# Keluaa/Armon.jl

Hardware: AMD Instinct MI355X
Metric: Mcells/sec per sweep (fp64) (higher is better)
Workload: dtype f64; 1 GPU; Sod 16384x16384 fp64, GAD+minmod+euler_2nd, Sequential X,Y splitting, nghost 4, 1x1 tiles of 16384x16384 cells (strong scaling); arithmetic=tuned (shared 1-ulp reciprocals + FMA; within the reference's golden tolerance), cells_per_gpu=268435456, transport=single block, device=AMD GPU gfx950 (gfx950:sramecc+:xnack-, 256 CUs), halo_exchange_downgraded=False, full=False

## Files before the change

### armon.jl_amd/csrc/common.hpp

```cpp
#pragma once

#include <hip/hip_runtime.h>

#include <cstdarg>
#include <cstdint>
#include <cstdio>
#include <cstring>

#include "../../include/armon_hip.h"

struct armon_graph;
struct armon_ctx {
    int device = 0;
    hipStream_t stream = nullptr;
    bool owns_stream = false;
    double* partials = nullptr;
    size_t partials_cap = 0;
    double* scalars = nullptr;
    double* host_scalars = nullptr;
    hipEvent_t ev_start = nullptr, ev_stop = nullptr;
    hipEvent_t* ev_pool = nullptr;
    int n_cu = 256;
    int tune_xs_niter = 0;
    int tune_y_seg = 0;
    int tune_align = 1;
    int tune_y_cols1 = 0;
    int tune_x_xcd = -1;
    int tune_x_rows = 0;
    int tune_copy_nt = 0;
    int tune_y_sx = 0;
    int64_t seg_nx = -1, seg_ny = -1;
    int seg_lag = -1, seg_cols = -1, seg_value = 0;
    int live_graphs = 0;
    armon_graph* graphs = nullptr;
    bool capturing = false;
};

namespace armon {

void set_error(const char* fmt, ...);

inline int fail_hip(hipError_t e, const char* what)
{
    set_error("%s: %s", what, hipGetErrorString(e));
    return ARMON_ERR_HIP;
}

#define ARMON_HIP_TRY(expr)                                             \
    do {                                                                \
        hipError_t e_ = (expr);                                         \
        if (e_ != hipSuccess) return ::armon::fail_hip(e_, #expr);      \
    } while (0)

#define ARMON_REQUIRE(cond, ...)                                        \
    do {                                                                \
        if (!(cond)) {                                                  \
            ::armon::set_error(__VA_ARGS__);                            \
            return ARMON_ERR_INVALID_ARG;                               \
        }                                                               \
    } while (0)

inline int check_launch(const char* name)
{
    hipError_t e = hipGetLastError();
    if (e != hipSuccess) {
// ... 30 lines not shown
```

### armon.jl_amd/csrc/context.hip

```cpp
#include "common.hpp"

#include <cstdlib>

namespace armon {

static thread_local char g_error[512] = "";

void set_error(const char* fmt, ...)
{
    va_list ap;
    va_start(ap, fmt);
    vsnprintf(g_error, sizeof(g_error), fmt, ap);
    va_end(ap);
}

int ensure_partials(armon_ctx* ctx, size_t n)
{
    if (n <= ctx->partials_cap) return ARMON_OK;
    ARMON_REQUIRE(!ctx->capturing, "the reduction scratch would have to grow (%zu -> %zu doubles) inside a stream capture: "
                  "run this launch once before armon_hip_graph_begin", ctx->partials_cap, n);
    ARMON_REQUIRE(ctx->live_graphs == 0, "the reduction scratch would have to grow (%zu -> %zu doubles) while %d captured graph(s) of "
                  "this context point into it: destroy them first, or run the larger launch before capturing",
                  ctx->partials_cap, n, ctx->live_graphs);
    ARMON_HIP_TRY(hipStreamSynchronize(ctx->stream));
// ... 37 lines not shown
        set_error("no HIP device available (%s)", e != hipSuccess ? hipGetErrorString(e) : "count = 0");
        return ARMON_ERR_NO_DEVICE;
    }
    ARMON_REQUIRE(device_id >= 0 && device_id < n, "device_id %d out of range [0,%d)", device_id, n);
    ARMON_HIP_TRY(hipSetDevice(device_id));

    hipDeviceProp_t prop;
    ARMON_HIP_TRY(hipGetDeviceProperties(&prop, device_id));
    if (strncmp(prop.gcnArchName, "gfx950", 6) != 0) {
        set_error("device %d is %s; this library holds gfx950 code objects only", device_id, prop.gcnArchName);
        return ARMON_ERR_NO_DEVICE;
    }

    armon_ctx* ctx = new armon_ctx();
    ctx->device = device_id;
    ctx->n_cu = prop.multiProcessorCount;
    if (stream) {
        ctx->stream = (hipStream_t)stream;
        ctx->owns_stream = false;
    } else {
        e = hipStreamCreateWithFlags(&ctx->stream, hipStreamNonBlocking);
        if (e != hipSuccess) { delete ctx; return fail_hip(e, "hipStreamCreate"); }
        ctx->owns_stream = true;
    }
    if ((e = hipMalloc((void**)&ctx->scalars, 16 * sizeof(double))) != hipSuccess ||
        (e = hipHostMalloc((void**)&ctx->host_scalars, 16 * sizeof(double), hipHostMallocDefault)) != hipSuccess ||
        (e = hipEventCreate(&ctx->ev_start)) != hipSuccess ||
        (e = hipEventCreate(&ctx->ev_stop)) != hipSuccess) {
        armon_hip_destroy(ctx);
        return fail_hip(e, "context allocation");
    }
    int rc = ensure_partials(ctx, 8192);
    if (rc != ARMON_OK) { armon_hip_destroy(ctx); return rc; }
    for (const char* knob : {"ARMON_XS_NITER", "ARMON_Y_SEG", "ARMON_SWEEP_ALIGN", "ARMON_Y_COLS1", "ARMON_X_XCD", "ARMON_X_ROWS", "ARMON_Y_SX", "ARMON_COPY_NT"}) {
        const char* v = getenv(knob);
        if (v && *v) (void)armon_hip_set_tuning(ctx, knob, atoi(v));
    }
    *out = ctx;
    return ARMON_OK;
}

int armon_hip_set_tuning(armon_ctx* ctx, const char* knob, int value)
{
    ARMON_REQUIRE(ctx && knob, "NULL argument");
    if (!strcmp(knob, "ARMON_XS_NITER")) ctx->tune_xs_niter = value > 0 ? value : 0;
    else if (!strcmp(knob, "ARMON_Y_SEG")) ctx->tune_y_seg = value > 0 ? value : 0;
    else if (!strcmp(knob, "ARMON_SWEEP_ALIGN")) ctx->tune_align = value < 0 ? 1 : (value != 0);
    else if (!strcmp(knob, "ARMON_Y_COLS1")) ctx->tune_y_cols1 = value > 0;
    else if (!strcmp(knob, "ARMON_X_XCD")) ctx->tune_x_xcd = value < 0 ? -1 : (value > 0);
    else if (!strcmp(knob, "ARMON_X_ROWS")) ctx->tune_x_rows = (value == 1 || value == 2) ? value : 0;
    else if (!strcmp(knob, "ARMON_Y_SX")) ctx->tune_y_sx = (value == 1 || value == 2) ? value : 0;
    else if (!strcmp(knob, "ARMON_COPY_NT")) ctx->tune_copy_nt = value & 3;
    else ARMON_REQUIRE(false, "unknown tuning knob '%s'", knob);
    return ARMON_OK;
}

int armon_hip_get_tuning(armon_ctx* ctx, const char* knob, int* value)
{
    ARMON_REQUIRE(ctx && knob && value, "NULL argument");
    if (!strcmp(knob, "ARMON_XS_NITER")) *value = ctx->tune_xs_niter;
    else if (!strcmp(knob, "ARMON_Y_SEG")) *value = ctx->tune_y_seg;
    else if (!strcmp(knob, "ARMON_SWEEP_ALIGN")) *value = ctx->tune_align;
    else if (!strcmp(knob, "ARMON_Y_COLS1")) *value = ctx->tune_y_cols1;
    else if (!strcmp(knob, "ARMON_X_XCD")) *value = ctx->tune_x_xcd;
    else if (!strcmp(knob, "ARMON_X_ROWS")) *value = ctx->tune_x_rows;
    else if (!strcmp(knob, "ARMON_Y_SX")) *value = ctx->tune_y_sx;
    else if (!strcmp(knob, "ARMON_COPY_NT")) *value = ctx->tune_copy_nt;
    else if (!strcmp(knob, "Y_RUN_ROWS")) *value = ctx->tune_y_seg > 0 ? ctx->tune_y_seg : ctx->seg_value;
    else ARMON_REQUIRE(false, "unknown tuning knob '%s'", knob);
    return ARMON_OK;
}

int armon_hip_destroy(armon_ctx* ctx)
{
    if (!ctx) return ARMON_OK;
    (void)hipSetDevice(ctx->device);
    if (ctx->stream) (void)hipStreamSynchronize(ctx->stream);
    disown_graphs(ctx);
    if (ctx->partials) (void)hipFree(ctx->partials);
    if (ctx->scalars) (void)hipFree(ctx->scalars);
    if (ctx->host_scalars) (void)hipHostFree(ctx->host_scalars);
    if (ctx->ev_pool) {
        for (int i = 0; i < ARMON_HIP_MAX_EVENTS; i++)
            if (ctx->ev_pool[i]) (void)hipEventDestroy(ctx->ev_pool[i]);
        delete[] ctx->ev_pool;
    }
    if (ctx->ev_start) (void)hipEventDestroy(ctx->ev_start);
    if (ctx->ev_stop) (void)hipEventDestroy(ctx->ev_stop);
    if (ctx->owns_stream && ctx->stream) (void)hipStreamDestroy(ctx->stream);
    delete ctx;
    return ARMON_OK;
}

int armon_hip_sync(armon_ctx* ctx)
{
    ARMON_REQUIRE(ctx, "ctx is NULL");
    ARMON_HIP_TRY(hipStreamSynchronize(ctx->stream));
// ... 200 lines not shown
```

### armon.jl_amd/csrc/fused_sweep_impl.hpp

```cpp
#pragma once
#include "common.hpp"
#include "dt_state.hpp"
#include "reduce.hpp"
#include "sweep_pipeline.hpp"
#include "sweep_spatial.hpp"

#include <cmath>
#include <cstdint>
#include <cstdlib>
#include <type_traits>
#include <utility>
#include <vector>

using namespace armon;

#ifndef ARMON_SWEEP_REAL
#error "include through fused_sweep_f64.hip / fused_sweep_f32.hip"
#endif

namespace {

using real = ARMON_SWEEP_REAL;
using vec2 = std::conditional<std::is_same<real, double>::value, double2, float2>::type;

// ... 8 lines not shown
#define ARMON_NT_Y 2
#endif
typedef real vreal2 __attribute__((ext_vector_type(2)));
template <bool NT = false>
__device__ __forceinline__ vec2 ld2(const real* p)
{
    const vreal2* q = reinterpret_cast<const vreal2*>(p);
    const vreal2 v = NT ? __builtin_nontemporal_load(q) : *q;
    return vec2{v.x, v.y};
}
constexpr bool x_nt_loads(int eos, bool exact)
{
    return (ARMON_NT_X & 1) && sizeof(real) == 8 && eos == ARMON_EOS_PERFECT_GAS && !exact;
}
__device__ __forceinline__ void st2(real* p, real x, real y)
{
    vreal2* q = reinterpret_cast<vreal2*>(p);
    const vreal2 v = {x, y};
    if (ARMON_NT_X & 2) __builtin_nontemporal_store(v, q);
    else *q = v;
}

struct sweep_args {
    int64_t nx, ny, row_len;
    int32_t g;
    int32_t bc_low, bc_high;
    int32_t emit;
    int32_t seg;
    int32_t x_kernel;
    int64_t o_lo, o_hi;
    int64_t x_first;
    int32_t xshift;
    int32_t xcd_remap;
    int32_t gx = 0, gy = 0;
    int32_t x_wg_along_x = 0;
    int32_t x_row_align = 0;
    int32_t y_sx = 0;
    armon_dt_state* st = nullptr;
    real dt, dx, gamma;
    real inv_dx, dt_dx;
    real fa_low, ft_low, fa_high, ft_high;
    const real *rho_in, *ua_in, *ut_in, *E_in;
    real *rho_out, *ua_out, *ut_out, *E_out;
    real *p_out, *c_out;
    real* partials;
    int32_t bc_low_t = 0, bc_high_t = 0;
    real tu_low = 1, tv_low = 1, tu_high = 1, tv_high = 1;
};

__device__ __forceinline__ int64_t bc_source(const sweep_args& a, int64_t n, int64_t j, real& fa, real& ft)
{
    fa = 1;
    ft = 1;
    if (j < 0 && a.bc_low) {
        fa = a.fa_low;
        ft = a.ft_low;
        return -1 - j;
    }
    if (j >= n && a.bc_high) {
        fa = a.fa_high;
        ft = a.ft_high;
        return 2 * n - 1 - j;
    }
    return j;
}

// ... 133 lines not shown
    }
}

int fold_dt_launch(armon_ctx* ctx, real* partials, int64_t n, real dx, real dy, real* out, int accumulate,
                   armon_dt_state* st = nullptr)
{
    if (n > 16384) {
        real* level1 = partials + 2 * n;
        hipLaunchKernelGGL(k_fold_pairs, dim3(kFoldBlocks), dim3(256), 0, ctx->stream, partials, n, level1);
        int rc = check_launch("fold_pairs");
        if (rc != ARMON_OK) return rc;
        partials = level1;
        n = kFoldBlocks;
    }
    hipLaunchKernelGGL(k_fold_dt, dim3(1), dim3(256), 0, ctx->stream, partials, n, dx, dy, out, accumulate, st);
    return check_launch("fold_dt");
}

#ifndef ARMON_Y_BLOCK
#define ARMON_Y_BLOCK 256
#endif
constexpr int kYBlock = ARMON_Y_BLOCK;
constexpr int kYSxBlock = 512;
#ifndef ARMON_Y_PF
#define ARMON_Y_PF 4
#endif
#ifndef ARMON_Y_PRIO
#define ARMON_Y_PRIO 0
#endif
#ifndef ARMON_Y_WAVES
#define ARMON_Y_WAVES 2
#endif

template <class PIPE, bool TRACK, int BLOCK = kYBlock, bool SX = false>
__global__ void __launch_bounds__(BLOCK, ARMON_Y_WAVES)
k_sweep_y(sweep_args a)
{
    if (!sweep_begin(a)) return;
    constexpr int LAG = PIPE::LAG;
    constexpr int PF = ARMON_Y_PF;
    const int nx = (int)a.nx, ny = (int)a.ny, g = a.g;
    const int xr = (int)(blockIdx.x * BLOCK + threadIdx.x) - a.xshift;
    const bool active = xr >= 0 && xr < nx;
    const int x = active ? xr : (xr < 0 ? 0 : nx - 1);
    const int o_hi = (int)a.o_hi;
    const int o0 = (int)a.o_lo + (int)blockIdx.y * a.seg;
    const int o1 = (o0 + a.seg < o_hi) ? o0 + a.seg : o_hi;
    const int jb = o0 - LAG, je = o1 + LAG;

    const unsigned colb = (unsigned)(x + g) * (unsigned)sizeof(real);
    const unsigned pitchb = (unsigned)a.row_len * (unsigned)sizeof(real);
    const int64_t in_base = (int64_t)(jb + g) * a.row_len, out_base = (int64_t)(o0 + g) * a.row_len;
    const rsrc_t r_rho = make_rsrc(a.rho_in + in_base), r_ua = make_rsrc(a.ua_in + in_base);
    const rsrc_t r_ut = make_rsrc(a.ut_in + in_base), r_E = make_rsrc(a.E_in + in_base);
    const rsrc_t w_rho = make_rsrc(a.rho_out + out_base), w_ua = make_rsrc(a.ua_out + out_base);
    const rsrc_t w_ut = make_rsrc(a.ut_out + out_base), w_E = make_rsrc(a.E_out + out_base);

    PIPE pipe(a.dt, a.dx, a.gamma, a.inv_dx, a.dt_dx);
    cfl_track cfl;

    int lj = jb;
    unsigned lo_off = 0;
    unsigned so_off = (unsigned)(jb - LAG - o0) * pitchb;

    __shared__ real sx_lds[SX ? 2 : 1][SX ? 4 : 1][SX ? BLOCK : 1];
    static_assert((BLOCK & (BLOCK - 1)) == 0, "the store exchange wraps columns with a mask");
    constexpr int kSec = 64 / (int)sizeof(real);
    const int c0 = (int)(blockIdx.x * BLOCK) - a.xshift;
    int sx_r = (int)(((int64_t)(jb - LAG + g) * a.row_len + g + c0) & (kSec - 1));
    const int sx_dr = (int)(a.row_len & (kSec - 1));
    int sx_buf = 0;

    auto load = [&](auto slot, auto checked) {
        constexpr int K = decltype(slot)::value & 7;
        constexpr bool CHECKED = decltype(checked)::value;
        auto& dst = pipe.c[K];
        if (CHECKED) {
            const bool m_lo = lj < 0 && a.bc_low, m_hi = lj >= ny && a.bc_high;
            const int src = m_lo ? -1 - lj : (m_hi ? 2 * ny - 1 - lj : lj);
            const unsigned off = (unsigned)(src - jb) * pitchb;
            const real fa = m_lo ? a.fa_low : (m_hi ? a.fa_high : real(1));
            const real ft = m_lo ? a.ft_low : (m_hi ? a.ft_high : real(1));
            dst.rho = buf_load<real>(r_rho, colb, off);
            dst.ua = buf_load<real>(r_ua, colb, off) * fa;
            dst.ut = buf_load<real>(r_ut, colb, off) * ft;
            dst.E = buf_load<real>(r_E, colb, off);
            if (lj + 1 < je) {
                lj++;
                lo_off += pitchb;
            }
        } else {
            dst.rho = buf_load<real>(r_rho, colb, lo_off);
            dst.ua = buf_load<real>(r_ua, colb, lo_off);
            dst.ut = buf_load<real>(r_ut, colb, lo_off);
            dst.E = buf_load<real>(r_E, colb, lo_off);
            lj++;
            lo_off += pitchb;
        }
    };
    using std::integral_constant;
    auto step = [&](auto ph, auto checked, int j) {
// ... 33 lines not shown
                const int ci = ((int)threadIdx.x - sx_r) & (BLOCK - 1);
                const int cx = c0 + ci;
                if (cx >= 0 && cx < nx) {
                    const unsigned cb = (unsigned)(cx + g) * (unsigned)sizeof(real);
                    buf_store(w_rho, cb, so_off, L[0][ci]);
                    buf_store(w_ua, cb, so_off, L[1][ci]);
                    buf_store(w_ut, cb, so_off, L[2][ci]);
                    buf_store(w_E, cb, so_off, L[3][ci]);
                }
                sx_buf ^= 1;
            } else if (active) {
                buf_store(w_rho, colb, so_off, out.rho);
                buf_store(w_ua, colb, so_off, out.ua);
                buf_store(w_ut, colb, so_off, out.ut);
                buf_store(w_E, colb, so_off, out.E);
            }
            if (TRACK) cfl.add(out.ut, out.ua, c_lag);
        }
        so_off += pitchb;
        sx_r = (sx_r + sx_dr) & (kSec - 1);
    };
    auto run = [&](auto checked, int t0, int t1) {
        for (int t = t0; t < t1; t += 8)
            static_for(std::make_integer_sequence<int, 8>{}, [&](auto ph) { step(ph, checked, jb + t + decltype(ph)::value); });
    };

    const int T = je - jb;
    const int T8 = (T + 7) & ~7;
    const int P = (2 * LAG + 7) & ~7;
    const int plain_end = (a.bc_high && ny < je ? ny : je) - jb - PF;
    int M = (T < plain_end ? T : plain_end) & ~7;
    if (M < P || (a.emit & 3)) M = P;

    const bool wave_idle = !SX && (int)(blockIdx.x * BLOCK + (threadIdx.x & ~63u)) - a.xshift >= nx;
    if (!wave_idle) {
        static_for(std::make_integer_sequence<int, PF>{}, [&](auto k) { load(k, std::true_type{}); });
        run(std::true_type{}, 0, P < T8 ? P : T8);
        run(std::false_type{}, P, M);
        run(std::true_type{}, M, T8);
    }

    if (TRACK) cfl_block_store<BLOCK / 64>(cfl, a.partials, (int64_t)blockIdx.y * gridDim.x + blockIdx.x, threadIdx.x);
}

template <class PIPE, bool TRACK, int BLOCK = kYBlock, bool SX = false>
__global__ void __launch_bounds__(BLOCK, ARMON_Y_WAVES)
k_sweep_y2(sweep_args a)
{
    if (!sweep_begin(a)) return;
    constexpr int LAG = PIPE::LAG;
    constexpr int PF = ARMON_Y_PF;
    const int nx = (int)a.nx, ny = (int)a.ny, g = a.g;
    const int xr = (int)(blockIdx.x * BLOCK + threadIdx.x) * 2 - a.xshift;
    const bool active = xr >= 0 && xr < nx;
    const int x = active ? xr : (xr < 0 ? 0 : nx - 2);
    const int o_hi = (int)a.o_hi;
    const int o0 = (int)a.o_lo + (int)blockIdx.y * a.seg;
    const int o1 = (o0 + a.seg < o_hi) ? o0 + a.seg : o_hi;
    const int jb = o0 - LAG, je = o1 + LAG;

    const unsigned colb = (unsigned)(x + g) * (unsigned)sizeof(real);
    const unsigned pitchb = (unsigned)a.row_len * (unsigned)sizeof(real);
    const int64_t in_base = (int64_t)(jb + g) * a.row_len, out_base = (int64_t)(o0 + g) * a.row_len;
    const rsrc_t r_rho = make_rsrc(a.rho_in + in_base), r_ua = make_rsrc(a.ua_in + in_base);
    const rsrc_t r_ut = make_rsrc(a.ut_in + in_base), r_E = make_rsrc(a.E_in + in_base);
    const rsrc_t w_rho = make_rsrc(a.rho_out + out_base), w_ua = make_rsrc(a.ua_out + out_base);
    const rsrc_t w_ut = make_rsrc(a.ut_out + out_base), w_E = make_rsrc(a.E_out + out_base);

    using V = fused::fast::float2v;
    using PIPEV = fused::PipeFast<PIPE::SCHEME, PIPE::LIM, PIPE::PROJ, PIPE::EOS, V>;
    PIPEV pipe(a.dt, a.dx, a.gamma, a.inv_dx, a.dt_dx);
    cfl_track cfl;

    int lj = jb;
    unsigned lo_off = 0;
    unsigned so_off = (unsigned)(jb - LAG - o0) * pitchb;

    __shared__ float2 sx_lds[SX ? 2 : 1][SX ? 4 : 1][SX ? BLOCK : 1];
    static_assert((BLOCK & (BLOCK - 1)) == 0, "the store exchange wraps columns with a mask");
    const int c0 = (int)(blockIdx.x * BLOCK) * 2 - a.xshift;
    int sx_r = (int)((((int64_t)(jb - LAG + g) * a.row_len + g + c0) >> 1) & 7);
    const int sx_dr = (int)((a.row_len >> 1) & 7);
    int sx_buf = 0;

    auto load = [&](auto slot, auto checked) {
        constexpr int K = decltype(slot)::value & 7;
        constexpr bool CHECKED = decltype(checked)::value;
        auto& dst = pipe.c[K];
        auto vec = [](float2 q) { return V{q.x, q.y}; };
        auto put = [&](unsigned off, real fa, real ft) {
            dst.rho = vec(buf_load2(r_rho, colb, off));
            dst.ua = vec(buf_load2(r_ua, colb, off)) * fa;
            dst.ut = vec(buf_load2(r_ut, colb, off)) * ft;
            dst.E = vec(buf_load2(r_E, colb, off));
        };
        if (CHECKED) {
            const bool m_lo = lj < 0 && a.bc_low, m_hi = lj >= ny && a.bc_high;
            const int src = m_lo ? -1 - lj : (m_hi ? 2 * ny - 1 - lj : lj);
            const unsigned off = (unsigned)(src - jb) * pitchb;
            const real fa = m_lo ? a.fa_low : (m_hi ? a.fa_high : real(1));
            const real ft = m_lo ? a.ft_low : (m_hi ? a.ft_high : real(1));
            put(off, fa, ft);
            if (lj + 1 < je) {
                lj++;
                lo_off += pitchb;
            }
        } else {
            dst.rho = vec(buf_load2(r_rho, colb, lo_off));
            dst.ua = vec(buf_load2(r_ua, colb, lo_off));
            dst.ut = vec(buf_load2(r_ut, colb, lo_off));
            dst.E = vec(buf_load2(r_E, colb, lo_off));
            lj++;
            lo_off += pitchb;
// ... 40 lines not shown
                }
                sx_buf ^= 1;
            } else if (active) {
                buf_store2(w_rho, colb, so_off, out.rho.x, out.rho.y);
                buf_store2(w_ua, colb, so_off, out.ua.x, out.ua.y);
                buf_store2(w_ut, colb, so_off, out.ut.x, out.ut.y);
                buf_store2(w_E, colb, so_off, out.E.x, out.E.y);
            }
            if (TRACK) {
                cfl.add(out.ut.x, out.ua.x, c_lag.x);
                cfl.add(out.ut.y, out.ua.y, c_lag.y);
            }
        }
        so_off += pitchb;
        sx_r = (sx_r + sx_dr) & 7;
    };
    auto run = [&](auto checked, int t0, int t1) {
        for (int t = t0; t < t1; t += 8)
            static_for(std::make_integer_sequence<int, 8>{}, [&](auto ph) { step(ph, checked, jb + t + decltype(ph)::value); });
    };

    const int T = je - jb;
    const int T8 = (T + 7) & ~7;
    const int P = (2 * LAG + 7) & ~7;
    const int plain_end = (a.bc_high && ny < je ? ny : je) - jb - PF;
    int M = (T < plain_end ? T : plain_end) & ~7;
    if (M < P || (a.emit & 3)) M = P;

    static_for(std::make_integer_sequence<int, PF>{}, [&](auto k) { load(k, std::true_type{}); });
    run(std::true_type{}, 0, P < T8 ? P : T8);
    run(std::false_type{}, P, M);
    run(std::true_type{}, M, T8);

    if (TRACK) cfl_block_store<BLOCK / 64>(cfl, a.partials, (int64_t)blockIdx.y * gridDim.x + blockIdx.x, threadIdx.x);
}

#ifndef ARMON_XS_ROWS
#define ARMON_XS_ROWS 4
#endif
constexpr int kXSRows = ARMON_XS_ROWS;
#ifndef ARMON_X_PRIO
#define ARMON_X_PRIO 3
#endif
constexpr int kXSNiter = 1;
template <int SCHEME, int LIM, int PROJ, int EOS, bool EXACT, int K, bool TRACK, bool SINGLE, int ROW = 0>
__device__ __forceinline__ void sweep_x_dpp_body(const sweep_args& a, int niter)
{
    using SW = fused::SpatialSweep<SCHEME, LIM, PROJ, EOS, EXACT, K, real, ROW>;
    using St = fused::Strip<K, real>;
    constexpr int LAG = SW::LAG;
    static_assert(ROW == 0 || K == 1, "the narrow form holds one cell per lane");
    constexpr int HALO = (K == 1) ? LAG : 4;
    static_assert(LAG <= 4, "strip halo");
    constexpr int WIDTH = ROW ? 16 : 64 * K;
    constexpr int STRIDE = WIDTH - 2 * HALO;
    constexpr int RW = ROW ? 4 : 1;

    const int lane = ROW ? (threadIdx.x & 15) : threadIdx.x;
    unsigned vbx = blockIdx.x, vby = blockIdx.y;
    if (a.xcd_remap) {
        const unsigned G = (unsigned)a.gx, chunk = vby & ~7u;
        if (chunk + 8 <= (unsigned)a.gy) {
            const unsigned local = (vby - chunk) * G + vbx;
            vby = chunk + (local & 7u);
            vbx = local >> 3;
        }
    }
// ... 136 lines not shown
__device__ __forceinline__ void preload_x_args(const sweep_args& a, int niter)
{
#if ARMON_X_PRELOAD
    asm volatile("" ::"s"(a.nx), "s"(a.ny), "s"(a.row_len), "s"(a.g), "s"(a.bc_low), "s"(a.bc_high), "s"(a.emit), "s"(a.o_lo),
                 "s"(a.o_hi), "s"(a.x_first), "s"(a.xcd_remap), "s"(a.x_wg_along_x), "s"(a.x_row_align), "s"(niter), "s"(a.gx), "s"(a.gy));
    asm volatile("" ::"s"(a.dt), "s"(a.dx), "s"(a.gamma), "s"(a.inv_dx), "s"(a.dt_dx), "s"(a.rho_in), "s"(a.ua_in), "s"(a.ut_in),
                 "s"(a.E_in), "s"(a.rho_out), "s"(a.ua_out), "s"(a.ut_out), "s"(a.E_out));
#endif
}

template <int SCHEME, int LIM, int PROJ, int EOS, bool EXACT, int K, bool TRACK, bool SINGLE = true, int ROW = 0>
__global__ void __launch_bounds__(64 * kXSRows, ARMON_XS_WAVES)
k_sweep_x_dpp(sweep_args a, int niter)
{
#if ARMON_X_PRIO
    __builtin_amdgcn_s_setprio(ARMON_X_PRIO);
#endif
    preload_x_args(a, niter);
    if (!sweep_begin(a)) return;
    sweep_x_dpp_body<SCHEME, LIM, PROJ, EOS, EXACT, K, TRACK, SINGLE, ROW>(a, niter);
}

#ifdef ARMON_ALT_KERNELS
#include "fused_sweep_alt_kernels.hpp"
#endif

template <class PIPE, bool TRACK>
int launch(armon_ctx* ctx, const sweep_args& a, int axis, int64_t* n_blocks)
{
    const int64_t n_out = a.o_hi - a.o_lo;
    if constexpr (std::is_same<real, float>::value && !PIPE::kExact) {
        if (axis == ARMON_AXIS_Y && a.nx % 2 == 0 && a.g % 2 == 0 && a.nx >= 2 && !ctx->tune_y_cols1) {
            const int block = a.y_sx ? kYSxBlock : kYBlock;
            dim3 grid((unsigned)((a.nx + a.xshift + 2 * block - 1) / (2 * block)), (unsigned)((n_out + a.seg - 1) / a.seg));
            *n_blocks = (int64_t)grid.x * grid.y;
            if (a.y_sx)
                hipLaunchKernelGGL((k_sweep_y2<PIPE, TRACK, kYSxBlock, true>), grid, dim3(block), 0, ctx->stream, a);
            else
                hipLaunchKernelGGL((k_sweep_y2<PIPE, TRACK>), grid, dim3(block), 0, ctx->stream, a);
            return check_launch("sweep_y2");
        }
    }
    if (axis == ARMON_AXIS_Y) {
        const int block = a.y_sx ? kYSxBlock : kYBlock;
        dim3 grid((unsigned)((a.nx + a.xshift + block - 1) / block), (unsigned)((n_out + a.seg - 1) / a.seg));
        *n_blocks = (int64_t)grid.x * grid.y;
        if constexpr (!PIPE::kExact) {
            if (a.y_sx) {
                hipLaunchKernelGGL((k_sweep_y<PIPE, TRACK, kYSxBlock, true>), grid, dim3(block), 0, ctx->stream, a);
                return check_launch("sweep_y (store exchange)");
            }
        }
        hipLaunchKernelGGL((k_sweep_y<PIPE, TRACK>), grid, dim3(block), 0, ctx->stream, a);
        return check_launch("sweep_y");
    }
#if defined(ARMON_ALT_KERNELS) && !defined(ARMON_ONLY_HEADLINE)
    if (a.x_kernel == 2) {
        dim3 grid((unsigned)((n_out + a.seg - 1) / a.seg), (unsigned)((a.ny + kXRows - 1) / kXRows));
        *n_blocks = (int64_t)grid.x * grid.y;
        const size_t lds = (size_t)(a.emit ? 6 : 4) * kXRows * (kXChunk + 1) * sizeof(real);
        hipLaunchKernelGGL((k_sweep_x_lds<PIPE, kXChunk, TRACK>), grid, dim3(kXRows), lds, ctx->stream, a);
        return check_launch("sweep_x_lds");
    }
#endif
    int niter = 1;
#if defined(ARMON_ALT_KERNELS) && !defined(ARMON_ONLY_HEADLINE)
    if (ctx->tune_xs_niter > 1) niter = ctx->tune_xs_niter;
#elif defined(ARMON_XS_MULTI)
    niter = ctx->tune_xs_niter > 0 ? ctx->tune_xs_niter : 2;
#endif
    const bool k1 = a.x_kernel == 3;
    if (a.x_kernel == 0 && a.o_hi - a.o_lo <= 8) {
        const int64_t per_block = 16 - 2 * PIPE::LAG;
        dim3 grid((unsigned)((a.o_hi - a.x_first + per_block - 1) / per_block), (unsigned)((a.ny + 4 * kXSRows - 1) / (4 * kXSRows)));
        *n_blocks = (int64_t)grid.x * grid.y * kXSRows;
        sweep_args b = a;
        b.gx = (int32_t)grid.x;
        b.gy = (int32_t)grid.y;
        hipLaunchKernelGGL((k_sweep_x_dpp<PIPE::SCHEME, PIPE::LIM, PIPE::PROJ, PIPE::EOS, PIPE::kExact, 1, TRACK, true, 1>),
                           grid, dim3(64, kXSRows), 0, ctx->stream, b, 1);
        return check_launch("sweep_x_dpp (narrow)");
    }
    const int halo = k1 ? PIPE::LAG : 4;
    const int64_t per_block = (int64_t)niter * (64 * (k1 ? 1 : 2) - 2 * halo);
    const int64_t x_lowest = a.x_row_align ? a.o_lo - (64 / (int64_t)sizeof(real) - 1) : a.x_first;
    dim3 grid((unsigned)((a.o_hi - x_lowest + per_block - 1) / per_block), (unsigned)((a.ny + kXSRows - 1) / kXSRows));
    if (a.x_wg_along_x && !k1 && niter == 1)
        grid = dim3((unsigned)((a.o_hi - x_lowest + kXSRows * per_block - 1) / (kXSRows * per_block)), (unsigned)a.ny);
    *n_blocks = (int64_t)grid.x * grid.y * kXSRows;
    sweep_args b = a;
    b.gx = (int32_t)grid.x;
    b.gy = (int32_t)grid.y;
#if defined(ARMON_ALT_KERNELS) && !defined(ARMON_ONLY_HEADLINE)
    if (k1)
        hipLaunchKernelGGL((k_sweep_x_dpp<PIPE::SCHEME, PIPE::LIM, PIPE::PROJ, PIPE::EOS, PIPE::kExact, 1, TRACK, false>),
                           grid, dim3(64, kXSRows), 0, ctx->stream, b, niter);
    else if (niter > 1)
        hipLaunchKernelGGL((k_sweep_x_dpp<PIPE::SCHEME, PIPE::LIM, PIPE::PROJ, PIPE::EOS, PIPE::kExact, 2, TRACK, false>),
                           grid, dim3(64, kXSRows), 0, ctx->stream, b, niter);
    else
#endif
#ifdef ARMON_XS_MULTI
        hipLaunchKernelGGL((k_sweep_x_dpp<PIPE::SCHEME, PIPE::LIM, PIPE::PROJ, PIPE::EOS, PIPE::kExact, 2, TRACK, false>),
                           grid, dim3(64, kXSRows), 0, ctx->stream, b, niter);
#else
        hipLaunchKernelGGL((k_sweep_x_dpp<PIPE::SCHEME, PIPE::LIM, PIPE::PROJ, PIPE::EOS, PIPE::kExact, 2, TRACK, true>),
                           grid, dim3(64, kXSRows), 0, ctx->stream, b, niter);
#endif
    return check_launch("sweep_x_dpp");
}

int y_run_length(int n_cu, int64_t nx, int64_t ny, int lag, int cols_per_lane, int block)
{
    const double slots = (double)n_cu * ARMON_Y_WAVES * 4 / (block / 64);
    const int64_t cols = (nx + 16 + (int64_t)block * cols_per_lane - 1) / ((int64_t)block * cols_per_lane);
    int best = (int)(ny < 32 ? ny : 32);
    double best_cost = 1e300;
    for (int64_t nruns = 1; nruns <= ny; nruns++) {
        const int64_t seg = (ny + nruns - 1) / nruns;
        if (seg < 32) break;
        if ((ny + seg - 1) / seg != nruns) continue;
        const double rounds = (double)(cols * nruns) / slots;
        const bool full_single_round = rounds <= 1. && rounds >= 0.93;
        if (rounds < 2. && !full_single_round) continue;
        const double cost = (full_single_round ? 1. : 0.5 * (rounds + std::ceil(rounds))) * (double)(seg + 2 * lag);
        if (cost < best_cost) {
            best_cost = cost;
            best = (int)seg;
        }
    }
    return best;
}

int64_t max_blocks(const sweep_args& a)
{
    const int64_t by = (a.nx + 16 + kYBlock - 1) / kYBlock * ((a.ny + a.seg - 1) / a.seg);
#ifdef ARMON_ALT_KERNELS
    const int64_t bx_lds = (a.nx + a.seg - 1) / a.seg * ((a.ny + kXRows - 1) / kXRows);
#else
    const int64_t bx_lds = 0;
#endif
    const int64_t bx_dpp = ((a.nx + 8) / 56 + 1 + kXSRows) * ((a.ny + kXSRows - 1) / kXSRows) * kXSRows;
    int64_t m = by > bx_lds ? by : bx_lds;
    m = m > bx_dpp ? m : bx_dpp;
    return m + kFoldBlocks;
}

template <class PIPE>
int dispatch_track(armon_ctx* ctx, const sweep_args& a, int axis, bool track, int64_t* n_blocks)
{
    if (track) return launch<PIPE, true>(ctx, a, axis, n_blocks);
    return launch<PIPE, false>(ctx, a, axis, n_blocks);
}

template <int SCHEME, int LIM, int PROJ, int EOS>
int dispatch_exact(armon_ctx* ctx, const sweep_args& a, int axis, bool exact, bool track, int64_t* nb)
{
    if (exact) return dispatch_track<fused::Pipe<SCHEME, LIM, PROJ, EOS, real>>(ctx, a, axis, track, nb);
// ... 56 lines not shown
    a.ny = d->ny;
    a.row_len = d->nx + 2 * (int64_t)d->nghost;
    a.g = d->nghost;
    a.bc_low = d->bc_low;
    a.bc_high = d->bc_high;
    a.emit = (d->p_out ? 1 : 0) | (d->c_out ? 2 : 0);
    a.dt = (real)d->dt;
    a.dx = (real)d->dx;
    a.gamma = (real)d->gamma;
    a.inv_dx = real(1) / a.dx;
    a.dt_dx = a.dt / a.dx;
    const bool X = d->axis == ARMON_AXIS_X;
    a.fa_low = (real)(X ? d->u_factor_low : d->v_factor_low);
    a.ft_low = (real)(X ? d->v_factor_low : d->u_factor_low);
    a.fa_high = (real)(X ? d->u_factor_high : d->v_factor_high);
    a.ft_high = (real)(X ? d->v_factor_high : d->u_factor_high);
    a.rho_in = d->rho_in;
    a.ua_in = X ? d->u_in : d->v_in;
    a.ut_in = X ? d->v_in : d->u_in;
    a.E_in = d->E_in;
    a.rho_out = d->rho_out;
    a.ua_out = X ? d->u_out : d->v_out;
    a.ut_out = X ? d->v_out : d->u_out;
    a.E_out = d->E_out;
    a.p_out = d->p_out;
    a.c_out = d->c_out;
    a.st = d->dt_state;
    const bool align = ctx->tune_align != 0;
    a.y_sx = 0;
    if (!X && align && ctx->tune_y_sx != 2 && !d->exact) {
        const uintptr_t outs = (uintptr_t)d->rho_out | (uintptr_t)d->u_out | (uintptr_t)d->v_out | (uintptr_t)d->E_out;
        a.y_sx = outs % 64 == 0 && ((a.row_len * (int64_t)sizeof(real)) % 64 != 0 || ctx->tune_y_sx == 1);
    }
    if (X) {
        a.seg = 512;
    } else if (ctx->tune_y_seg > 0) {
        a.seg = ctx->tune_y_seg;
    } else {
        const int cols_per_lane = (std::is_same<real, float>::value && !d->exact && d->nx % 2 == 0 && d->nghost % 2 == 0 &&
                                   d->nx >= 2 && !ctx->tune_y_cols1) ? 2 : 1;
        const int y_block = a.y_sx ? kYSxBlock : kYBlock;
        if (ctx->seg_nx != d->nx || ctx->seg_ny != n_axis || ctx->seg_lag != lag || ctx->seg_cols != cols_per_lane * y_block) {
            ctx->seg_value = y_run_length(ctx->n_cu, d->nx, n_axis, lag, cols_per_lane, y_block);
            ctx->seg_cols = cols_per_lane * y_block;
            ctx->seg_nx = d->nx;
            ctx->seg_ny = n_axis;
            ctx->seg_lag = lag;
        }
        a.seg = ctx->seg_value;
    }
    ARMON_REQUIRE(X || a.row_len * (int64_t)sizeof(real) * (a.seg + 2 * lag + 16) < (1ll << 32),
                  "block too wide for 32-bit row offsets (%lld cells per row, runs of %d rows)", (long long)d->nx, a.seg);
    a.x_kernel = d->x_kernel;
    a.o_lo = 0;
    a.o_hi = n_axis;
    if (d->out_hi != 0) {
        ARMON_REQUIRE(d->out_lo >= 0 && d->out_lo < d->out_hi && d->out_hi <= n_axis,
                      "invalid partial sweep [%lld, %lld) of %lld cells", (long long)d->out_lo, (long long)d->out_hi, (long long)n_axis);
        a.o_lo = d->out_lo;
        a.o_hi = d->out_hi;
    }
    a.xshift = (X || !align) ? 0 : d->nghost % 16;
    a.x_first = X ? (align ? a.o_lo - (a.o_lo + d->nghost) % 8 : a.o_lo) : 0;
    const bool want_along_x = ctx->tune_x_rows == 2 || (ctx->tune_x_rows == 0 && sizeof(real) == 4);
    const bool along_x = X && want_along_x && d->ny <= 65535 && ctx->tune_x_xcd <= 0;
    const bool eight_xcds = ctx->n_cu == 256;
    a.xcd_remap = (ctx->tune_x_xcd < 0 ? sizeof(real) == 8 : ctx->tune_x_xcd != 0) && !along_x && eight_xcds;
    a.x_row_align = 0;
#ifndef ARMON_XS_MULTI
    {
        const uintptr_t bases = (uintptr_t)d->rho_in | (uintptr_t)d->u_in | (uintptr_t)d->v_in | (uintptr_t)d->E_in |
                                (uintptr_t)d->rho_out | (uintptr_t)d->u_out | (uintptr_t)d->v_out | (uintptr_t)d->E_out |
                                (uintptr_t)d->p_out | (uintptr_t)d->c_out;
        a.x_row_align = X && align && d->x_kernel == 0 && ctx->tune_xs_niter <= 1 && a.row_len % (64 / (int64_t)sizeof(real)) != 0 &&
                        bases % 64 == 0;
    }
#endif
    a.x_wg_along_x = along_x ? 1 : 0;
    a.partials = nullptr;
    if (track) {
        int rc = ensure_partials(ctx, (size_t)(2 * max_blocks(a)));
        if (rc != ARMON_OK) return rc;
        a.partials = reinterpret_cast<real*>(ctx->partials);
    }

    int64_t n_blocks = 0;
    int rc;
#ifdef ARMON_ONLY_HEADLINE
#ifndef ARMON_ONLY_EOS
#define ARMON_ONLY_EOS ARMON_EOS_PERFECT_GAS
#endif
    ARMON_REQUIRE(d->scheme == ARMON_SCHEME_GAD && d->limiter == ARMON_LIMITER_MINMOD && d->projection == ARMON_PROJECTION_EULER_2ND &&
                  d->eos == ARMON_ONLY_EOS && d->x_kernel == 0, "headline-only variant build");
    rc = dispatch_exact<ARMON_SCHEME_GAD, ARMON_LIMITER_MINMOD, ARMON_PROJECTION_EULER_2ND, ARMON_ONLY_EOS>(ctx, a, d->axis, exact, track, &n_blocks);
    if (rc != ARMON_OK || !track) return rc;
    return fold_dt_launch(ctx, a.partials, n_blocks, (real)d->cfl_dx, (real)d->cfl_dy, d->dt_cfl_out, d->dt_accumulate, d->dt_state);
#else
    if (d->scheme == ARMON_SCHEME_GODUNOV) {
        rc = dispatch_proj<ARMON_SCHEME_GODUNOV, ARMON_LIMITER_NONE>(ctx, a, d->axis, d->eos, d->projection, exact, track, &n_blocks);
    } else {
// ... 184 lines not shown
```

Baseline: 96710 Mcells/s.

## Remap Y-sweep workgroups across XCDs and wrap leftover columns into first block

```diff
diff --git a/armon.jl_amd/csrc/common.hpp b/armon.jl_amd/csrc/common.hpp
--- a/armon.jl_amd/csrc/common.hpp
+++ b/armon.jl_amd/csrc/common.hpp
@@ -26,11 +26,13 @@
     int tune_align = 1;
     int tune_y_cols1 = 0;
     int tune_x_xcd = -1;
+    int tune_y_xcd = -1;
+    int tune_y_wrap = -1;
     int tune_x_rows = 0;
     int tune_copy_nt = 0;
     int tune_y_sx = 0;
     int64_t seg_nx = -1, seg_ny = -1;
-    int seg_lag = -1, seg_cols = -1, seg_value = 0;
+    int seg_lag = -1, seg_cols = -1, seg_wrap = -1, seg_value = 0;
     int live_graphs = 0;
     armon_graph* graphs = nullptr;
     bool capturing = false;
diff --git a/armon.jl_amd/csrc/context.hip b/armon.jl_amd/csrc/context.hip
--- a/armon.jl_amd/csrc/context.hip
+++ b/armon.jl_amd/csrc/context.hip
@@ -93,7 +93,8 @@
     }
     int rc = ensure_partials(ctx, 8192);
     if (rc != ARMON_OK) { armon_hip_destroy(ctx); return rc; }
-    for (const char* knob : {"ARMON_XS_NITER", "ARMON_Y_SEG", "ARMON_SWEEP_ALIGN", "ARMON_Y_COLS1", "ARMON_X_XCD", "ARMON_X_ROWS", "ARMON_Y_SX", "ARMON_COPY_NT"}) {
+    for (const char* knob : {"ARMON_XS_NITER", "ARMON_Y_SEG", "ARMON_SWEEP_ALIGN", "ARMON_Y_COLS1", "ARMON_X_XCD", "ARMON_Y_XCD", "ARMON_X_ROWS",
+                             "ARMON_Y_SX", "ARMON_Y_WRAP", "ARMON_COPY_NT"}) {
         const char* v = getenv(knob);
         if (v && *v) (void)armon_hip_set_tuning(ctx, knob, atoi(v));
     }
@@ -109,6 +110,8 @@
     else if (!strcmp(knob, "ARMON_SWEEP_ALIGN")) ctx->tune_align = value < 0 ? 1 : (value != 0);
     else if (!strcmp(knob, "ARMON_Y_COLS1")) ctx->tune_y_cols1 = value > 0;
     else if (!strcmp(knob, "ARMON_X_XCD")) ctx->tune_x_xcd = value < 0 ? -1 : (value > 0);
+    else if (!strcmp(knob, "ARMON_Y_XCD")) ctx->tune_y_xcd = value < 0 ? -1 : (value > 0);
+    else if (!strcmp(knob, "ARMON_Y_WRAP")) ctx->tune_y_wrap = value < 0 ? -1 : (value > 0);
     else if (!strcmp(knob, "ARMON_X_ROWS")) ctx->tune_x_rows = (value == 1 || value == 2) ? value : 0;
     else if (!strcmp(knob, "ARMON_Y_SX")) ctx->tune_y_sx = (value == 1 || value == 2) ? value : 0;
     else if (!strcmp(knob, "ARMON_COPY_NT")) ctx->tune_copy_nt = value & 3;
@@ -124,6 +127,8 @@
     else if (!strcmp(knob, "ARMON_SWEEP_ALIGN")) *value = ctx->tune_align;
     else if (!strcmp(knob, "ARMON_Y_COLS1")) *value = ctx->tune_y_cols1;
     else if (!strcmp(knob, "ARMON_X_XCD")) *value = ctx->tune_x_xcd;
+    else if (!strcmp(knob, "ARMON_Y_XCD")) *value = ctx->tune_y_xcd;
+    else if (!strcmp(knob, "ARMON_Y_WRAP")) *value = ctx->tune_y_wrap;
     else if (!strcmp(knob, "ARMON_X_ROWS")) *value = ctx->tune_x_rows;
     else if (!strcmp(knob, "ARMON_Y_SX")) *value = ctx->tune_y_sx;
     else if (!strcmp(knob, "ARMON_COPY_NT")) *value = ctx->tune_copy_nt;
diff --git a/armon.jl_amd/csrc/fused_sweep_impl.hpp b/armon.jl_amd/csrc/fused_sweep_impl.hpp
--- a/armon.jl_amd/csrc/fused_sweep_impl.hpp
+++ b/armon.jl_amd/csrc/fused_sweep_impl.hpp
@@ -64,6 +64,8 @@
     int64_t x_first;
     int32_t xshift;
     int32_t xcd_remap;
+    int32_t y_xcd = 0;
+    int32_t y_wrap = 0;
     int32_t gx = 0, gy = 0;
     int32_t x_wg_along_x = 0;
     int32_t x_row_align = 0;
@@ -263,6 +265,22 @@
 #define ARMON_Y_WAVES 2
 #endif
 
+__device__ __forceinline__ void y_block_coords(const sweep_args& a, unsigned& bx, unsigned& by)
+{
+    bx = blockIdx.x;
+    by = blockIdx.y;
+    if (a.y_xcd) {
+        const unsigned G = (unsigned)a.gx, chunk = by & ~7u;
+        const unsigned rows = (unsigned)a.gy - chunk < 8u ? (unsigned)a.gy - chunk : 8u;
+        const unsigned n = rows * G, id = (by - chunk) * G + bx;
+        const unsigned k = id & 7u, q = n >> 3, r = n & 7u;
+        const unsigned v = k * q + (k < r ? k : r) + (id >> 3);
+        const unsigned dy = (unsigned)__builtin_amdgcn_readfirstlane((int)(v / G));
+        by = chunk + dy;
+        bx = v - dy * G;
+    }
+}
+
 template <class PIPE, bool TRACK, int BLOCK = kYBlock, bool SX = false>
 __global__ void __launch_bounds__(BLOCK, ARMON_Y_WAVES)
 k_sweep_y(sweep_args a)
@@ -271,11 +289,14 @@
     constexpr int LAG = PIPE::LAG;
     constexpr int PF = ARMON_Y_PF;
     const int nx = (int)a.nx, ny = (int)a.ny, g = a.g;
-    const int xr = (int)(blockIdx.x * BLOCK + threadIdx.x) - a.xshift;
+    unsigned bx, by;
+    y_block_coords(a, bx, by);
+    const int xr0 = (int)(bx * BLOCK + threadIdx.x) - a.xshift;
+    const int xr = (xr0 < 0 && xr0 >= -a.y_wrap) ? nx + xr0 : xr0;
     const bool active = xr >= 0 && xr < nx;
     const int x = active ? xr : (xr < 0 ? 0 : nx - 1);
     const int o_hi = (int)a.o_hi;
-    const int o0 = (int)a.o_lo + (int)blockIdx.y * a.seg;
+    const int o0 = (int)a.o_lo + (int)by * a.seg;
     const int o1 = (o0 + a.seg < o_hi) ? o0 + a.seg : o_hi;
     const int jb = o0 - LAG, je = o1 + LAG;
 
@@ -297,7 +318,7 @@
     __shared__ real sx_lds[SX ? 2 : 1][SX ? 4 : 1][SX ? BLOCK : 1];
     static_assert((BLOCK & (BLOCK - 1)) == 0, "the store exchange wraps columns with a mask");
     constexpr int kSec = 64 / (int)sizeof(real);
-    const int c0 = (int)(blockIdx.x * BLOCK) - a.xshift;
+    const int c0 = (int)(bx * BLOCK) - a.xshift;
     int sx_r = (int)(((int64_t)(jb - LAG + g) * a.row_len + g + c0) & (kSec - 1));
     const int sx_dr = (int)(a.row_len & (kSec - 1));
     int sx_buf = 0;
@@ -397,7 +418,7 @@
     int M = (T < plain_end ? T : plain_end) & ~7;
     if (M < P || (a.emit & 3)) M = P;
 
-    const bool wave_idle = !SX && (int)(blockIdx.x * BLOCK + (threadIdx.x & ~63u)) - a.xshift >= nx;
+    const bool wave_idle = !SX && (int)(bx * BLOCK + (threadIdx.x & ~63u)) - a.xshift >= nx;
     if (!wave_idle) {
         static_for(std::make_integer_sequence<int, PF>{}, [&](auto k) { load(k, std::true_type{}); });
         run(std::true_type{}, 0, P < T8 ? P : T8);
@@ -405,7 +426,7 @@
         run(std::true_type{}, M, T8);
     }
 
-    if (TRACK) cfl_block_store<BLOCK / 64>(cfl, a.partials, (int64_t)blockIdx.y * gridDim.x + blockIdx.x, threadIdx.x);
+    if (TRACK) cfl_block_store<BLOCK / 64>(cfl, a.partials, (int64_t)blockIdx.y * a.gx + blockIdx.x, threadIdx.x);
 }
 
 template <class PIPE, bool TRACK, int BLOCK = kYBlock, bool SX = false>
@@ -416,11 +437,14 @@
     constexpr int LAG = PIPE::LAG;
     constexpr int PF = ARMON_Y_PF;
     const int nx = (int)a.nx, ny = (int)a.ny, g = a.g;
-    const int xr = (int)(blockIdx.x * BLOCK + threadIdx.x) * 2 - a.xshift;
+    unsigned bx, by;
+    y_block_coords(a, bx, by);
+    const int xr0 = (int)(bx * BLOCK + threadIdx.x) * 2 - a.xshift;
+    const int xr = (xr0 < 0 && xr0 >= -a.y_wrap) ? nx + xr0 : xr0;
     const bool active = xr >= 0 && xr < nx;
     const int x = active ? xr : (xr < 0 ? 0 : nx - 2);
     const int o_hi = (int)a.o_hi;
-    const int o0 = (int)a.o_lo + (int)blockIdx.y * a.seg;
+    const int o0 = (int)a.o_lo + (int)by * a.seg;
     const int o1 = (o0 + a.seg < o_hi) ? o0 + a.seg : o_hi;
     const int jb = o0 - LAG, je = o1 + LAG;
 
@@ -443,7 +467,7 @@
 
     __shared__ float2 sx_lds[SX ? 2 : 1][SX ? 4 : 1][SX ? BLOCK : 1];
     static_assert((BLOCK & (BLOCK - 1)) == 0, "the store exchange wraps columns with a mask");
-    const int c0 = (int)(blockIdx.x * BLOCK) * 2 - a.xshift;
+    const int c0 = (int)(bx * BLOCK) * 2 - a.xshift;
     int sx_r = (int)((((int64_t)(jb - LAG + g) * a.row_len + g + c0) >> 1) & 7);
     const int sx_dr = (int)((a.row_len >> 1) & 7);
     int sx_buf = 0;
@@ -550,7 +574,7 @@
     run(std::false_type{}, P, M);
     run(std::true_type{}, M, T8);
 
-    if (TRACK) cfl_block_store<BLOCK / 64>(cfl, a.partials, (int64_t)blockIdx.y * gridDim.x + blockIdx.x, threadIdx.x);
+    if (TRACK) cfl_block_store<BLOCK / 64>(cfl, a.partials, (int64_t)blockIdx.y * a.gx + blockIdx.x, threadIdx.x);
 }
 
 #ifndef ARMON_XS_ROWS
@@ -753,26 +777,32 @@
     if constexpr (std::is_same<real, float>::value && !PIPE::kExact) {
         if (axis == ARMON_AXIS_Y && a.nx % 2 == 0 && a.g % 2 == 0 && a.nx >= 2 && !ctx->tune_y_cols1) {
             const int block = a.y_sx ? kYSxBlock : kYBlock;
-            dim3 grid((unsigned)((a.nx + a.xshift + 2 * block - 1) / (2 * block)), (unsigned)((n_out + a.seg - 1) / a.seg));
+            dim3 grid((unsigned)((a.nx + a.xshift - a.y_wrap + 2 * block - 1) / (2 * block)), (unsigned)((n_out + a.seg - 1) / a.seg));
             *n_blocks = (int64_t)grid.x * grid.y;
+            sweep_args b = a;
+            b.gx = (int32_t)grid.x;
+            b.gy = (int32_t)grid.y;
             if (a.y_sx)
-                hipLaunchKernelGGL((k_sweep_y2<PIPE, TRACK, kYSxBlock, true>), grid, dim3(block), 0, ctx->stream, a);
+                hipLaunchKernelGGL((k_sweep_y2<PIPE, TRACK, kYSxBlock, true>), grid, dim3(block), 0, ctx->stream, b);
             else
-                hipLaunchKernelGGL((k_sweep_y2<PIPE, TRACK>), grid, dim3(block), 0, ctx->stream, a);
+                hipLaunchKernelGGL((k_sweep_y2<PIPE, TRACK>), grid, dim3(block), 0, ctx->stream, b);
             return check_launch("sweep_y2");
         }
     }
     if (axis == ARMON_AXIS_Y) {
         const int block = a.y_sx ? kYSxBlock : kYBlock;
-        dim3 grid((unsigned)((a.nx + a.xshift + block - 1) / block), (unsigned)((n_out + a.seg - 1) / a.seg));
+        dim3 grid((unsigned)((a.nx + a.xshift - a.y_wrap + block - 1) / block), (unsigned)((n_out + a.seg - 1) / a.seg));
         *n_blocks = (int64_t)grid.x * grid.y;
+        sweep_args b = a;
+        b.gx = (int32_t)grid.x;
+        b.gy = (int32_t)grid.y;
         if constexpr (!PIPE::kExact) {
             if (a.y_sx) {
-                hipLaunchKernelGGL((k_sweep_y<PIPE, TRACK, kYSxBlock, true>), grid, dim3(block), 0, ctx->stream, a);
+                hipLaunchKernelGGL((k_sweep_y<PIPE, TRACK, kYSxBlock, true>), grid, dim3(block), 0, ctx->stream, b);
                 return check_launch("sweep_y (store exchange)");
             }
         }
-        hipLaunchKernelGGL((k_sweep_y<PIPE, TRACK>), grid, dim3(block), 0, ctx->stream, a);
+        hipLaunchKernelGGL((k_sweep_y<PIPE, TRACK>), grid, dim3(block), 0, ctx->stream, b);
         return check_launch("sweep_y");
     }
 #if defined(ARMON_ALT_KERNELS) && !defined(ARMON_ONLY_HEADLINE)
@@ -831,10 +861,10 @@
     return check_launch("sweep_x_dpp");
 }
 
-int y_run_length(int n_cu, int64_t nx, int64_t ny, int lag, int cols_per_lane, int block)
+int y_run_length(int n_cu, int64_t nx, int64_t ny, int lag, int cols_per_lane, int block, bool wrap)
 {
     const double slots = (double)n_cu * ARMON_Y_WAVES * 4 / (block / 64);
-    const int64_t cols = (nx + 16 + (int64_t)block * cols_per_lane - 1) / ((int64_t)block * cols_per_lane);
+    const int64_t cols = (nx + 16 + (int64_t)block * cols_per_lane - 1) / ((int64_t)block * cols_per_lane) - (wrap ? 1 : 0);
     int best = (int)(ny < 32 ? ny : 32);
     double best_cost = 1e300;
     for (int64_t nruns = 1; nruns <= ny; nruns++) {
@@ -844,7 +874,8 @@
         const double rounds = (double)(cols * nruns) / slots;
         const bool full_single_round = rounds <= 1. && rounds >= 0.93;
         if (rounds < 2. && !full_single_round) continue;
-        const double cost = (full_single_round ? 1. : 0.5 * (rounds + std::ceil(rounds))) * (double)(seg + 2 * lag);
+        double cost = (full_single_round ? 1. : 0.5 * (rounds + std::ceil(rounds))) * (double)(seg + 2 * lag);
+        if (wrap) cost += 0.02 * (double)seg;
         if (cost < best_cost) {
             best_cost = cost;
             best = (int)seg;
@@ -967,20 +998,29 @@
         const uintptr_t outs = (uintptr_t)d->rho_out | (uintptr_t)d->u_out | (uintptr_t)d->v_out | (uintptr_t)d->E_out;
         a.y_sx = outs % 64 == 0 && ((a.row_len * (int64_t)sizeof(real)) % 64 != 0 || ctx->tune_y_sx == 1);
     }
+    a.xshift = (X || !align) ? 0 : d->nghost % 16;
+    const int cols_per_lane = (std::is_same<real, float>::value && !d->exact && d->nx % 2 == 0 && d->nghost % 2 == 0 &&
+                               d->nx >= 2 && !ctx->tune_y_cols1) ? 2 : 1;
+    const int y_block = a.y_sx ? kYSxBlock : kYBlock;
+    a.y_wrap = 0;
+    if (!X && !a.y_sx && (ctx->tune_y_wrap < 0 ? sizeof(real) == 8 : ctx->tune_y_wrap != 0)) {
+        const int64_t wg_cols = (int64_t)cols_per_lane * y_block, left = (d->nx + a.xshift) % wg_cols;
+        if (left > 0 && left <= a.xshift && d->nx + a.xshift > wg_cols && left % cols_per_lane == 0) a.y_wrap = (int32_t)left;
+    }
     if (X) {
         a.seg = 512;
     } else if (ctx->tune_y_seg > 0) {
         a.seg = ctx->tune_y_seg;
     } else {
-        const int cols_per_lane = (std::is_same<real, float>::value && !d->exact && d->nx % 2 == 0 && d->nghost % 2 == 0 &&
-                                   d->nx >= 2 && !ctx->tune_y_cols1) ? 2 : 1;
-        const int y_block = a.y_sx ? kYSxBlock : kYBlock;
-        if (ctx->seg_nx != d->nx || ctx->seg_ny != n_axis || ctx->seg_lag != lag || ctx->seg_cols != cols_per_lane * y_block) {
-            ctx->seg_value = y_run_length(ctx->n_cu, d->nx, n_axis, lag, cols_per_lane, y_block);
+        const int wrap = a.y_wrap ? 1 : 0;
+        if (ctx->seg_nx != d->nx || ctx->seg_ny != n_axis || ctx->seg_lag != lag || ctx->seg_cols != cols_per_lane * y_block ||
+            ctx->seg_wrap != wrap) {
+            ctx->seg_value = y_run_length(ctx->n_cu, d->nx, n_axis, lag, cols_per_lane, y_block, wrap);
             ctx->seg_cols = cols_per_lane * y_block;
             ctx->seg_nx = d->nx;
             ctx->seg_ny = n_axis;
             ctx->seg_lag = lag;
+            ctx->seg_wrap = wrap;
         }
         a.seg = ctx->seg_value;
     }
@@ -995,12 +1035,12 @@
         a.o_lo = d->out_lo;
         a.o_hi = d->out_hi;
     }
-    a.xshift = (X || !align) ? 0 : d->nghost % 16;
-    a.x_first = X ? (align ? a.o_lo - (a.o_lo + d->nghost) % 8 : a.o_lo) : 0;
+    a.x_first = X ?(align ? a.o_lo - (a.o_lo + d->nghost) % 8 : a.o_lo) : 0;
     const bool want_along_x = ctx->tune_x_rows == 2 || (ctx->tune_x_rows == 0 && sizeof(real) == 4);
     const bool along_x = X && want_along_x && d->ny <= 65535 && ctx->tune_x_xcd <= 0;
     const bool eight_xcds = ctx->n_cu == 256;
     a.xcd_remap = (ctx->tune_x_xcd < 0 ? sizeof(real) == 8 : ctx->tune_x_xcd != 0) && !along_x && eight_xcds;
+    a.y_xcd = !X && (ctx->tune_y_xcd < 0 ? sizeof(real) == 8 : ctx->tune_y_xcd != 0) && eight_xcds;
     a.x_row_align = 0;
 #ifndef ARMON_XS_MULTI
     {
```

Result: no change. 96660 Mcells/s (median of 2 runs) (-0.1%).
